# stone-d-chen/ffvvc

Measured on AMD Instinct MI355X. Metric: decoded frames/sec (4K/8K 10-bit VVC) per GPU, higher is better.
Workload: dtype u16

## Files before the change

ffvvc_amd/csrc/inter_cu.hip:

```cpp
#include <utility>

#include "common.hpp"
#include "inter_weight.hpp"
#include "runtime.hpp"
#include "../../include/vvc_mi355.h"
#include "stage_checks.hpp"

namespace vvc355 {

static_assert(sizeof(vvc355_affine_cu) == 144 && offsetof(vvc355_affine_cu, diff_mv) == 16 && offsetof(vvc355_affine_cu, first_job) == 12,
              "vvc355_affine_cu layout");
static_assert(sizeof(vvc355_gpm_cu) == 64 && offsetof(vvc355_gpm_cu, gpm_mv) == 16 && offsetof(vvc355_gpm_cu, first_job) == 12,
              "vvc355_gpm_cu layout");
static_assert(sizeof(vvc355_inter_frame) == 136, "vvc355_inter_frame layout");
static_assert(sizeof(vvc355_affine_frame) == 168 && offsetof(vvc355_affine_frame, cus) == 136 && offsetof(vvc355_affine_frame, n_cus) == 160,
              "vvc355_affine_frame layout");
static_assert(sizeof(vvc355_gpm_frame) == 160 && offsetof(vvc355_gpm_frame, cus) == 136 && offsetof(vvc355_gpm_frame, n_cus) == 152,
              "vvc355_gpm_frame layout");
static_assert(sizeof(vvc355_affine_job) == 96 && sizeof(vvc355_bipred_job) == 104 && sizeof(vvc355_gpm_job) == 120, "job layouts");
static_assert(sizeof(vvc355_ciip_cu) == 32 && offsetof(vvc355_ciip_cu, first_job) == 12 && offsetof(vvc355_ciip_cu, cmd) == 20, "vvc355_ciip_cu layout");
static_assert(sizeof(vvc355_ciip_frame) == 224 && offsetof(vvc355_ciip_frame, cus) == 136 && offsetof(vvc355_ciip_frame, n_cus) == 192 &&
              offsetof(vvc355_ciip_frame, ctb_log2) == 220, "vvc355_ciip_frame layout");
static_assert(sizeof(vvc355_recon_cmd) == 40 && offsetof(vvc355_recon_cmd, joint) == 33, "vvc355_recon_cmd layout");

void ciip_pred_launch(hipStream_t stream, int bd, const vvc355_bipred_job *jobs_dev, int n_jobs);

#define VVC355_TABLE(type, name, count) static constexpr type c_##name[count]
#include "tables_small.inc"
#undef VVC355_TABLE
#define VVC355_TABLE(type, name, count) __device__ static const type t_##name[count]
#include "tables_small.inc"
#undef VVC355_TABLE


constexpr int kGpmMaskSize = 112;
struct GpmMask { uint8_t w[kGpmMaskSize * kGpmMaskSize]; };

constexpr uint32_t gpm_used_angles()
{
    uint32_t m = 0;
    for (int p = 0; p < 64; p++) m |= 1u << c_gpm_angle_idx[p];
    return m;
}
constexpr uint32_t kGpmAngles = gpm_used_angles();
constexpr int kGpmMasks = __builtin_popcount(kGpmAngles);
static_assert(kGpmMasks == 20, "GPM uses 20 of the 32 angles");
__host__ __device__ constexpr int gpm_mask_slot(int angle) { return __builtin_popcount(kGpmAngles & ((1u << angle) - 1)); }
constexpr int gpm_slot_angle(int slot)
{
    for (int a = 0; a < 32; a++)
        if (((kGpmAngles >> a) & 1) && gpm_mask_slot(a) == slot) return a;
    return -1;
}

constexpr GpmMask make_gpm_mask(int angle)
{
    GpmMask m = {};
    const int dx = c_gpm_distance_lut[angle], dy = c_gpm_distance_lut[(angle + 8) % 32];
    const bool flip = !(angle >= 13 && angle <= 27);
    for (int v = 0; v < kGpmMaskSize; v++) {
        const int ry = (2 * (v - 56) + 1) * dy;
        for (int u = 0; u < kGpmMaskSize; u++) {
            const int idx = (2 * (u - 56) + 1) * dx + ry;
            const int s = ((flip ? 32 + idx : 32 - idx) + 4) >> 3;
            m.w[v * kGpmMaskSize + u] = (uint8_t)(s < 0 ? 0 : s > 8 ? 8 : s);
        }
    }
    return m;
}
template <int A> constexpr GpmMask kGpmMaskOf = make_gpm_mask(A);

template <typename Seq> struct GpmMaskSet;
template <size_t... S> struct GpmMaskSet<std::index_sequence<S...>> { GpmMask m[sizeof...(S)]; };
using GpmMaskTable = GpmMaskSet<std::make_index_sequence<kGpmMasks>>;
template <size_t... S> constexpr GpmMaskSet<std::index_sequence<S...>> make_gpm_masks(std::index_sequence<S...>)
{
    return { { kGpmMaskOf<gpm_slot_angle(S)>... } };
}
__device__ const GpmMaskTable d_gpm_masks = make_gpm_masks(std::make_index_sequence<kGpmMasks>{});
static const GpmMaskTable h_gpm_masks = make_gpm_masks(std::make_index_sequence<kGpmMasks>{});

struct GpmAddr { int slot, first, step_x, step_y; };
__host__ __device__ inline GpmAddr gpm_address(int angle, int distance, int cb_width, int cb_height, int hs, int vs)
{
    GpmAddr a;
    a.slot = gpm_mask_slot(angle);
    const bool shift_hor = !(angle % 16 == 8 || (angle % 16 != 0 && cb_height >= cb_width));
    int off_x = (-cb_width) >> 1, off_y = (-cb_height) >> 1;
    if (shift_hor)
        off_x += angle < 16 ? (distance * cb_width) >> 3 : -((distance * cb_width) >> 3);
    else
        off_y += angle < 16 ? (distance * cb_height) >> 3 : -((distance * cb_height) >> 3);
    const bool ok = cb_width >= 8 && cb_width <= 64 && cb_height >= 8 && cb_height <= 64 && ((kGpmAngles >> angle) & 1);
    a.first = ok ? (off_y + 56) * kGpmMaskSize + off_x + 56 : 0;
    a.step_x = ok ? 1 << hs : 0;
    a.step_y = ok ? kGpmMaskSize << vs : 0;
    return a;
}


template <typename Cu> __device__ __forceinline__ int find_cu(const Cu *cus, int n_cus, uint32_t i)
{
    int lo = 0, hi = n_cus - 1;
    while (lo < hi) {
        const int mid = (lo + hi + 1) >> 1;
        if (cus[mid].first_job <= i) lo = mid; else hi = mid - 1;
    }
    return lo;
}

__device__ __forceinline__ uint64_t plane_at(const vvc355_inter_frame &f, int c, int x, int y)
{
    return f.dst[c] + (uint64_t)y * f.dst_stride[c] + ((uint64_t)x << f.pixel_shift);
}

__device__ __forceinline__ int32_t round_mv_half(int32_t v) { return (v + 1 - (v >= 0)) >> 1; }

__global__ __launch_bounds__(256) void affine_build_kernel(const vvc355_affine_frame *__restrict__ fp)
{
    const vvc355_affine_frame F = load_uniform(fp);
    const vvc355_inter_frame &f = F.pic;
    const uint32_t i = blockIdx.x * blockDim.x + threadIdx.x;
    if (i >= (uint32_t)F.n_jobs)
        return;
    const vvc355_affine_cu *cus = (const vvc355_affine_cu *)F.cus;
    const int u = find_cu(cus, F.n_cus, i);
    const vvc355_affine_cu *cu = cus + u;
    const int x0 = cu->x0, y0 = cu->y0, cbw = cu->cb_width, cbh = cu->cb_height, nsx = cu->num_sb_x, nsy = cu->num_sb_y;
    const uint32_t first = cu->first_job;
    const uint32_t n_local = (u + 1 < F.n_cus ? cus[u + 1].first_job : (uint32_t)F.n_jobs) - first;
    const uint32_t k = i - first;
    const int hs = f.hs, vs = f.vs, csh = hs + vs;
    vvc355_affine_job *jl = (vvc355_affine_job *)F.jobs_luma;
    vvc355_bipred_job *jc = (vvc355_bipred_job *)F.jobs_chroma;
    const uint32_t cfirst = first >> csh;

    if (nsx != cbw >> 2 || nsy != cbh >> 2 || cbw < 8 || cbh < 8 || n_local != (uint32_t)(nsx * nsy)) {
        jl[i] = vvc355_affine_job{};
        if (f.chroma_format_idc && k < (n_local >> csh)) {
            jc[2 * (cfirst + k)] = vvc355_bipred_job{};
            jc[2 * (cfirst + k) + 1] = vvc355_bipred_job{};
        }
        return;
    }
    const vvc355_inter_slice *sl = (const vvc355_inter_slice *)f.slices + cu->slice;
    const vvc355_ref_pic *refs = (const vvc355_ref_pic *)f.refs;
    const MvFieldDev *mvf_tab = (const MvFieldDev *)f.mvf;
    const int sbx = k % nsx, sby = k / nsx;
    const int x = x0 + 4 * sbx, y = y0 + 4 * sby;
    const MvFieldDev mv = mvf_tab[(y >> 2) * f.mvf_stride + (x >> 2)];

    vvc355_affine_job j = {};
    j.dst = plane_at(f, 0, x, y);
    j.dst_stride = f.dst_stride[0];
    for (int l = 0; l < 2; l++) {
        if (!(mv.pred_flag & (1 << l)))
            continue;
        const vvc355_ref_pic rp = refs[l * 16 + mv.ref_idx[l]];
        (l ? j.ref1 : j.ref0) = rp.plane[0];
        (l ? j.ref1_stride : j.ref0_stride) = rp.stride[0];
        j.mv[2 * l] = mv.mv[l][0];
        j.mv[2 * l + 1] = mv.mv[l][1];
    }
    j.diff_mv = F.cus + (uint64_t)u * sizeof(vvc355_affine_cu) + offsetof(vvc355_affine_cu, diff_mv);
    j.x = (int16_t)x; j.y = (int16_t)y; j.pic_w = (int16_t)f.width; j.pic_h = (int16_t)f.height;
    set_pred_weight(j, derive_pred_weight(sl, mv, 0, false, false));
    j.pred_flag = mv.pred_flag;
    j.prof0 = cu->prof_flags & 1;
    j.prof1 = (cu->prof_flags >> 1) & 1;
    j.lmcs_lut = sl->lmcs_used ? f.lmcs_fwd_lut : 0;
    jl[i] = j;

    if (!f.chroma_format_idc || (sbx & ((1 << hs) - 1)) || (sby & ((1 << vs) - 1)))
        return;
    const MvFieldDev mv2 = mvf_tab[((y + vs * 4) >> 2) * f.mvf_stride + ((x + hs * 4) >> 2)];
    MvFieldDev mvc = mv;
    for (int l = 0; l < 2; l++)
        for (int d = 0; d < 2; d++)
// ... 82 lines not shown
    const vvc355_inter_frame &f = F.pic;
    const uint32_t i = blockIdx.x * blockDim.x + threadIdx.x;
    if (i >= (uint32_t)F.n_jobs)
        return;
    vvc355_bipred_job *slot = (vvc355_bipred_job *)F.jobs + i;
    vvc355_bipred_job j = {};
    const vvc355_ciip_cu *cus = (const vvc355_ciip_cu *)F.cus;
    const int u = find_cu(cus, F.n_cus, i);
    const vvc355_ciip_cu cu = cus[u];
    const int x0 = cu.x0, y0 = cu.y0, cbw = cu.cb_width, cbh = cu.cb_height, ctb_log2 = F.ctb_log2;
    const bool side_ok = cbw >= 4 && cbw <= 64 && !(cbw & (cbw - 1)) && cbh >= 4 && cbh <= 64 && !(cbh & (cbh - 1)) && cbw * cbh >= 64;
    const bool inside = x0 >= 0 && y0 >= 0 && !((x0 | y0) & 3) && x0 + cbw <= f.width && y0 + cbh <= f.height &&
                        (x0 >> ctb_log2) == ((x0 + cbw - 1) >> ctb_log2) && (y0 >> ctb_log2) == ((y0 + cbh - 1) >> ctb_log2);
    const bool has_c = f.chroma_format_idc != 0;
    const int wc = cbw >> f.hs, hc = cbh >> f.vs;
    const bool blend_c = has_c && wc > 2;
    const uint32_t ntl = ((cbw + 15) >> 4) * ((cbh + 15) >> 4), ntc = has_c ? ((wc + 15) >> 4) * ((hc + 15) >> 4) : 0;
    const uint32_t region = cbw * cbh + (blend_c ? 2 * wc * hc : 0);
    uint32_t k = i - cu.first_job;
    if (!side_ok || !inside || i < cu.first_job || cu.slice >= F.n_slices || (uint64_t)cu.first_job + ntl + 2 * ntc > (uint64_t)(uint32_t)F.n_jobs ||
        (uint64_t)cu.scratch_off + region > (uint64_t)(uint32_t)F.scratch_len || k >= ntl + 2 * ntc) {
        *slot = j;
        return;
    }
    const MvFieldDev *mvf_tab = (const MvFieldDev *)f.mvf;
    const MvFieldDev mv = mvf_tab[(y0 >> 2) * f.mvf_stride + (x0 >> 2)];
    bool mv_ok = mv.pred_flag >= 1 && mv.pred_flag <= 3;
    for (int l = 0; l < 2; l++)
        mv_ok = mv_ok && (!(mv.pred_flag & (1 << l)) || (mv.ref_idx[l] >= 0 && mv.ref_idx[l] <= 15));
    if (!mv_ok) {
        *slot = j;
        return;
    }
    const vvc355_inter_slice *sl = (const vvc355_inter_slice *)f.slices + cu.slice;
    const vvc355_ref_pic *refs = (const vvc355_ref_pic *)f.refs;
    int c = 0;
    if (k >= ntl) {
        k -= ntl;
        c = 1;
        if (k >= ntc) { k -= ntc; c = 2; }
    }
    const int hs = c ? f.hs : 0, vs = c ? f.vs : 0;
    const int w = cbw >> hs, h = cbh >> vs, tw = min(w, 16), th = min(h, 16);
    const int ntx = (w + 15) >> 4;
    const int tx = (k % ntx) * tw, ty = (k / ntx) * th;
    const int x = (x0 >> hs) + tx, y = (y0 >> vs) + ty;
    const bool to_plane = c && !blend_c;
    const uint64_t part = F.scratch + (((uint64_t)cu.scratch_off + (c ? cbw * cbh + (c - 1) * wc * hc : 0)) << f.pixel_shift);

    if (to_plane) {
        j.dst_stride = c == 1 ? f.dst_stride[1] : f.dst_stride[2];
        j.dst = (c == 1 ? f.dst[1] : f.dst[2]) + (uint64_t)y * j.dst_stride + ((uint64_t)x << f.pixel_shift);
    } else {
        j.dst = part + ((uint64_t)(ty * w + tx) << f.pixel_shift);
        j.dst_stride = w << f.pixel_shift;
    }
    for (int l = 0; l < 2; l++) {
        if (!(mv.pred_flag & (1 << l)))
            continue;
        const vvc355_ref_pic *rp = refs + l * 16 + mv.ref_idx[l];
        (l ? j.ref1 : j.ref0) = rp->plane[c];
        (l ? j.ref1_stride : j.ref0_stride) = rp->stride[c];
        j.mv[2 * l] = mv.mv[l][0];
        j.mv[2 * l + 1] = mv.mv[l][1];
    }
    j.x = (int16_t)x; j.y = (int16_t)y; j.w = (int16_t)tw; j.h = (int16_t)th;
    j.pic_w = (int16_t)(f.width >> hs); j.pic_h = (int16_t)(f.height >> vs);
    j.chroma = c > 0; j.hs = f.hs; j.vs = f.vs;
    j.hf_idx = j.vf_idx = c ? 0 : cu.hpel_if_idx & 1;
    j.pred_flag = mv.pred_flag;
    j.lmcs_lut = (!c && sl->lmcs_used) ? f.lmcs_fwd_lut : 0;
    set_pred_weight(j, derive_pred_weight(sl, mv, c, false, true));
    *slot = j;

    if (!F.cmds || k || to_plane)
        return;
    const uint32_t ci = cus[u].cmd[c];
    if (ci >= (uint32_t)F.n_cmds)
        return;
    vvc355_recon_cmd *cmd = (vvc355_recon_cmd *)F.cmds + ci;
    if (cmd->kind != VVC355_RECON_CIIP || cmd->c_idx != c || cmd->x0 != x0 || cmd->y0 != y0 || cmd->w != cbw || cmd->h != cbh)
        return;
    const int16_t *slice_idx = (const int16_t *)F.slice_idx, *col_bd = (const int16_t *)F.ctb_to_col_bd, *row_bd = (const int16_t *)F.ctb_to_row_bd;
    const int rx = x0 >> ctb_log2, ry = y0 >> ctb_log2, ncx = F.ctb_width, rs = ry * ncx + rx, ctb_mask = (1 << ctb_log2) - 1;
    const bool left_tile = rx > 0 && col_bd[rx] != col_bd[rx - 1];
    const bool upper_tile = ry > 0 && row_bd[ry] != row_bd[ry - 1];
    const bool upper_slice = ry > 0 && slice_idx[rs] != slice_idx[rs - ncx];
    const bool ctb_left = rx > 0 && !left_tile, ctb_up = ry > 0 && !upper_tile && !upper_slice;
    const bool available_l = ctb_left || (x0 & ctb_mask), available_u = ctb_up || (y0 & ctb_mask);
    int weight = 1;
    if (available_u && mvf_tab[((y0 - 1) >> 2) * f.mvf_stride + ((x0 - 1 + cbw) >> 2)].pred_flag == 0)
        weight++;
    if (available_l && mvf_tab[((y0 - 1 + cbh) >> 2) * f.mvf_stride + ((x0 - 1) >> 2)].pred_flag == 0)
        weight++;
    cmd->resid = part;
    cmd->joint = (uint8_t)weight;
}

int ciip_frame_check(const vvc355_ciip_frame *F, int bd)
{
    if (!F)
        return VVC355_CIIP_E_FRAME;
    const vvc355_inter_frame &f = F->pic;
    if (f.width <= 0 || f.height <= 0 || (f.width & 3) || (f.height & 3))
        return VVC355_CIIP_E_SIZE;
    if (F->ctb_log2 < 5 || F->ctb_log2 > 7)
        return VVC355_CIIP_E_CTB;
    const int ctb = 1 << F->ctb_log2;
    if (F->ctb_width != (f.width + ctb - 1) >> F->ctb_log2 || F->ctb_height != (f.height + ctb - 1) >> F->ctb_log2)
        return VVC355_CIIP_E_GRID;
    if (F->n_cus < 0 || F->n_jobs < 0 || F->scratch_len < 0 || F->n_slices < 0 || F->n_cmds < 0)
        return VVC355_CIIP_E_COUNT;
    if (bd >= 0 && ((bd != 8 && bd != 10 && bd != 12) || f.pixel_shift != (bd > 8)))
        return VVC355_CIIP_E_DEPTH;
    if (bd < 0 && f.pixel_shift > 1)
        return VVC355_CIIP_E_DEPTH;
    const int fmt_hs[4] = { 0, 1, 1, 0 }, fmt_vs[4] = { 0, 1, 0, 0 };
    if (f.chroma_format_idc > 3 || f.hs != fmt_hs[f.chroma_format_idc] || f.vs != fmt_vs[f.chroma_format_idc])
        return VVC355_CIIP_E_FORMAT;
    if (F->n_cus > 0 && !F->cus)
        return VVC355_CIIP_E_RECORDS;
    if (F->n_jobs > 0 && !F->jobs)
        return VVC355_CIIP_E_JOBS;
    if (!F->scratch || !f.mvf || !f.refs || !f.slices || !f.dst[0] || (f.chroma_format_idc && (!f.dst[1] || !f.dst[2])) || f.mvf_stride < f.width / 4)
        return VVC355_CIIP_E_TABLES;
    if (F->cmds && (!F->slice_idx || !F->ctb_to_col_bd || !F->ctb_to_row_bd))
        return VVC355_CIIP_E_CMDS;
    return 0;
}

}

extern "C" {

void vvc355_affine_frame_build(void *stream, const vvc355_affine_frame *frame_dev, const vvc355_affine_frame *frame_host)
{
    if (frame_host->n_cus <= 0 || frame_host->n_jobs <= 0) return;
    hipLaunchKernelGGL(vvc355::affine_build_kernel, dim3((frame_host->n_jobs + 255) / 256), dim3(256), 0, (hipStream_t)stream, frame_dev);
    HIP_CHECK(hipGetLastError());
}

void vvc355_affine_frame_pass(void *stream, int bd, const vvc355_affine_frame *frame_dev, const vvc355_affine_frame *frame_host)
{
    if (frame_host->n_cus <= 0 || frame_host->n_jobs <= 0) return;
    vvc355_affine_frame_build(stream, frame_dev, frame_host);
    vvc355_affine_frame_predict(stream, bd, frame_dev, frame_host);
}

void vvc355_affine_frame_predict(void *stream, int bd, const vvc355_affine_frame *, const vvc355_affine_frame *frame_host)
{
    if (frame_host->n_cus <= 0 || frame_host->n_jobs <= 0) return;
    vvc355_affine_batch(stream, bd, (const vvc355_affine_job *)frame_host->jobs_luma, frame_host->n_jobs);
    if (frame_host->pic.chroma_format_idc)
        vvc355_bipred_chroma_batch(stream, bd, (const vvc355_bipred_job *)frame_host->jobs_chroma,
                                   2 * (frame_host->n_jobs >> (frame_host->pic.hs + frame_host->pic.vs)));
}

void vvc355_gpm_frame_build(void *stream, const vvc355_gpm_frame *frame_dev, const vvc355_gpm_frame *frame_host)
{
    if (frame_host->n_cus <= 0 || frame_host->n_jobs <= 0) return;
    hipLaunchKernelGGL(vvc355::gpm_build_kernel, dim3((frame_host->n_jobs + 255) / 256), dim3(256), 0, (hipStream_t)stream, frame_dev);
    HIP_CHECK(hipGetLastError());
}

void vvc355_gpm_frame_pass(void *stream, int bd, const vvc355_gpm_frame *frame_dev, const vvc355_gpm_frame *frame_host)
{
    if (frame_host->n_cus <= 0 || frame_host->n_jobs <= 0) return;
    vvc355_gpm_frame_build(stream, frame_dev, frame_host);
    vvc355_gpm_frame_predict(stream, bd, frame_dev, frame_host);
}

void vvc355_gpm_frame_predict(void *stream, int bd, const vvc355_gpm_frame *, const vvc355_gpm_frame *frame_host)
{
    if (frame_host->n_cus <= 0 || frame_host->n_jobs <= 0) return;
    vvc355_gpm_batch(stream, bd, (const vvc355_gpm_job *)frame_host->jobs, frame_host->n_jobs);
}

int vvc355_ciip_frame_build(void *stream, const vvc355_ciip_frame *frame_dev, const vvc355_ciip_frame *frame_host)
{
    const int err = frame_dev ? vvc355::ciip_frame_check(frame_host, -1) : VVC355_CIIP_E_FRAME;
    if (err)
        return err;
    if (frame_host->n_cus == 0 || frame_host->n_jobs == 0) return 0;
    hipLaunchKernelGGL(vvc355::ciip_build_kernel, dim3((frame_host->n_jobs + 255) / 256), dim3(256), 0, (hipStream_t)stream, frame_dev);
    HIP_CHECK(hipGetLastError());
    return 0;
}

int vvc355_ciip_frame_pass(void *stream, int bd, const vvc355_ciip_frame *frame_dev, const vvc355_ciip_frame *frame_host)
{
    const int err = frame_dev ? vvc355::ciip_frame_check(frame_host, bd) : VVC355_CIIP_E_FRAME;
    if (err)
        return err;
    if (frame_host->n_cus == 0 || frame_host->n_jobs == 0) return 0;
    vvc355_ciip_frame_build(stream, frame_dev, frame_host);
    return vvc355_ciip_frame_predict(stream, bd, frame_dev, frame_host);
}

int vvc355_ciip_frame_predict(void *stream, int bd, const vvc355_ciip_frame *frame_dev, const vvc355_ciip_frame *frame_host)
{
    const int err = frame_dev ? vvc355::ciip_frame_check(frame_host, bd) : VVC355_CIIP_E_FRAME;
    if (err)
        return err;
    if (frame_host->n_cus == 0 || frame_host->n_jobs == 0) return 0;
    vvc355::ciip_pred_launch((hipStream_t)stream, bd, (const vvc355_bipred_job *)frame_host->jobs, frame_host->n_jobs);
    return 0;
}

void vvc355_gpm_weights(int partition_idx, int cb_width, int cb_height, int hs, int vs, uint8_t *out)
{
    using namespace vvc355;
    const int part = partition_idx & 63;
    const GpmAddr a = gpm_address(c_gpm_angle_idx[part], c_gpm_distance_idx[part], cb_width, cb_height, hs, vs);
    const uint8_t *m = h_gpm_masks.m[a.slot].w;
    const int w = cb_width >> hs, h = cb_height >> vs;
    for (int y = 0; y < h; y++)
        for (int x = 0; x < w; x++)
            out[y * w + x] = m[a.first + y * a.step_y + x * a.step_x];
}

}
```

ffvvc_amd/csrc/mc_fused.hip:

```cpp
#include <type_traits>
#include "common.hpp"
#include "runtime.hpp"
#include "../../include/vvc_mi355.h"

namespace vvc355 {

#define VVC355_TABLE(type, name, count) __device__ static const type d_tab_##name[count]
#include "tables.inc"
#undef VVC355_TABLE

typedef short v2s __attribute__((ext_vector_type(2)));

__device__ __forceinline__ int dot2(uint32_t a, uint32_t b, int acc)
{
    return __builtin_amdgcn_sdot2(__builtin_bit_cast(v2s, a), __builtin_bit_cast(v2s, b), acc, false);
}
__device__ __forceinline__ uint32_t pack16(int lo, int hi) { return (uint32_t)(lo & 0xffff) | ((uint32_t)hi << 16); }
__device__ __forceinline__ int tap_of(uint32_t lo, uint32_t hi, int k)
{
    const uint32_t v = k < 4 ? lo : hi;
    return (int)(int8_t)(v >> ((k & 3) * 8));
}

static constexpr int kWinW = 24;
// ... 320 lines not shown
            uint16_t r0[NIT], r1[NIT];
            fetch_clamped<BD, NIT>(pa, sa, g.rc[0], ax, ay, lane, r0);
            if (both)
                fetch_clamped<BD, NIT>(pb, sb, g.rc[1], bx, by, lane, r1);
            store_rows<NIT>(L.win[0], lane, r0);
            if (both)
                store_rows<NIT>(L.win[1], lane, r1);
        }
        wave_sync();
    }
    uint32_t t[2][4];
#pragma unroll
    for (int i = 0; i < 2; i++) {
        if (NTAP == 8) {
            const uint2 hf = gld<uint2>(d_tab_inter_luma_filters + (job->hf_idx * 16 + g.fx[i]) * 8);
            const uint2 vf = gld<uint2>(d_tab_inter_luma_filters + (job->vf_idx * 16 + g.fy[i]) * 8);
            t[i][0] = hf.x; t[i][1] = hf.y; t[i][2] = vf.x; t[i][3] = vf.y;
        } else {
            t[i][0] = gld<uint32_t>(d_tab_inter_chroma_filters + (job->hf_idx * 32 + g.fx[i]) * 4); t[i][1] = 0;
            t[i][2] = gld<uint32_t>(d_tab_inter_chroma_filters + (job->vf_idx * 32 + g.fy[i]) * 4); t[i][3] = 0;
        }
    }
    interp_block<BD, NTAP>(lw, h, g.fx[0] != 0, g.fy[0] != 0, t[0][0], t[0][1], t[0][2], t[0][3], L.win[0], L.tmpT, lane, v0);
    if (both)
        interp_block<BD, NTAP>(lw, h, g.fx[1] != 0, g.fy[1] != 0, t[1][0], t[1][1], t[1][2], t[1][3], L.win[1], L.tmpT, lane, v1);
    else {
#pragma unroll
        for (int i = 0; i < 4; i++) v1[i] = 0;
    }
}

#include "mc_tools.hpp"

union BipredLdsAll {
    BipredLds plain;
    ToolsLds<16, 16> tools;
};

template <int BD>
__device__ __forceinline__ void bipred_plain(const vvc355_bipred_job *job, BipredLds &L, int lane, const vvc355_gpm_job *gpm = nullptr)
{
    const int uni = job->pred_flag == 1 || job->pred_flag == 2;
    const int w = job->w, h = job->h, chroma = job->chroma;
    const int lw = 31 - __builtin_clz(w);
    vvc355_bipred_result *rec = (vvc355_bipred_result *)job->rec;
    int mv[4] = { job->mv[0], job->mv[1], job->mv[2], job->mv[3] };
    if (rec && chroma) {
#pragma unroll
        for (int k = 0; k < 4; k++) mv[k] = gld<int>(&rec->mv[k]);
    } else if (rec && lane == 0) {
#pragma unroll
        for (int k = 0; k < 4; k++) gst<int>(&rec->mv[k], mv[k]);
        gst<int>(&rec->bdof, 0);
        gst<int>(&rec->min_sad, 0);
        gst<int>(&rec->searched, 0);
    }
    RefGeom g = ref_geometry(job, mv, chroma, chroma && job->dmvr && !uni);
    const uint8_t *lut = chroma ? nullptr : (const uint8_t *)job->lmcs_lut;
    int v0[4], v1[4];
    const uint8_t *pa = (const uint8_t *)job->ref0, *pb = (const uint8_t *)job->ref1;
    int sa = job->ref0_stride, sb = job->ref1_stride;
    if (uni && job->pred_flag == 2) {
        pa = pb; sa = sb;
        g.ox[0] = g.ox[1]; g.oy[0] = g.oy[1]; g.fx[0] = g.fx[1]; g.fy[0] = g.fy[1]; g.rc[0] = g.rc[1];
    }
    if (chroma)
        predict_clamped<BD, 4>(job, L, lane, lw, h, g, v0, v1, pa, sa, pb, sb, !uni);
    else
        predict_clamped<BD, 8>(job, L, lane, lw, h, g, v0, v1, pa, sa, pb, sb, !uni);
    if (uni) {
        const int wfu = job->weight_flag, sh = (wfu ? job->denom : 0) + 14 - BD, rnd = 1 << (sh - 1);
        const int xu = lane & 15;
        uint8_t *dstu = (uint8_t *)job->dst;
#pragma unroll
        for (int i = 0; i < 4; i++) {
            const int y = 2 * ((lane >> 4) + 4 * (i >> 1)) + (i & 1);
            if (xu >= w || y >= h)
                continue;
            const int p = wfu ? ((v0[i] * job->w0 + rnd) >> sh) + job->o0 * (1 << (BD - 8)) : (v0[i] + rnd) >> sh;
            gst_at<typename Px<BD>::type>(dstu, (uint32_t)(__mul24(y, job->dst_stride) + xu * (int)sizeof(typename Px<BD>::type)), (typename Px<BD>::type)lmcs_fwd<BD>(lut, clip_px<BD>(p)));
        }
        return;
    }
#pragma unroll
    for (int i = 0; i < 4; i++) { v0[i] = (int16_t)v0[i]; v1[i] = (int16_t)v1[i]; }
    if (gpm) {
        constexpr int gsh = BD <= 12 ? 17 - BD : 5, goff = 1 << (gsh - 1);
        const uint8_t *wt = (const uint8_t *)gpm->weights;
        const int xg = lane & 15;
        uint8_t *dstg = (uint8_t *)job->dst;
#pragma unroll
        for (int i = 0; i < 4; i++) {
            const int y = 2 * ((lane >> 4) + 4 * (i >> 1)) + (i & 1);
            if (xg >= w || y >= h)
                continue;
            const int wg = gld<uint8_t>(wt + y * gpm->step_y + xg * gpm->step_x);
            const int p = (v0[i] * wg + v1[i] * (8 - wg) + goff) >> gsh;
            gst_at<typename Px<BD>::type>(dstg, (uint32_t)(__mul24(y, job->dst_stride) + xg * (int)sizeof(typename Px<BD>::type)), (typename Px<BD>::type)lmcs_fwd<BD>(lut, clip_px<BD>(p)));
        }
        return;
    }
    int shift, off;
    const int wf = job->weight_flag, w0 = job->w0, w1 = job->w1;
    if (!wf) { shift = max(3, 15 - BD); off = 1 << (shift - 1); }
    else     { shift = job->denom + max(3, 15 - BD); off = (((job->o0 + job->o1) << (BD - 8)) + 1) << (shift - 1); }
    const int x = lane & 15;
    uint8_t *dst = (uint8_t *)job->dst;
#pragma unroll
    for (int i = 0; i < 4; i++) {
        const int y = 2 * ((lane >> 4) + 4 * (i >> 1)) + (i & 1);
        if (x >= w || y >= h)
            continue;
        const int p = wf ? (v0[i] * w0 + v1[i] * w1 + off) >> shift : (v0[i] + v1[i] + off) >> shift;
        gst_at<typename Px<BD>::type>(dst, (uint32_t)(__mul24(y, job->dst_stride) + x * (int)sizeof(typename Px<BD>::type)), (typename Px<BD>::type)lmcs_fwd<BD>(lut, clip_px<BD>(p)));
    }
}

template <int BD, bool TOOLS>
__global__ __launch_bounds__(256) void bipred_kernel(const vvc355_bipred_job *__restrict__ jobs, int n_jobs)
{
    __shared__ __attribute__((aligned(16))) BipredLdsAll lds_all[4];
    const int wave = __builtin_amdgcn_readfirstlane(threadIdx.x >> 6), lane = threadIdx.x & 63;
    const int ji = xcd_chunked(blockIdx.x, gridDim.x) * 4 + wave;
    if (ji >= n_jobs)
        return;
    const vvc355_bipred_job job_copy = load_uniform(jobs + ji);
    const vvc355_bipred_job *job = &job_copy;
    BipredLdsAll &L = lds_all[wave];
    const int w = job->w, h = job->h, uni = job->pred_flag == 1 || job->pred_flag == 2;
    if (TOOLS && !job->chroma && !uni && (job->dmvr || job->bdof) && (w == 8 || w == 16) && (h == 8 || h == 16)) {
        if (w == 16 && h == 16)     bipred_tools<BD, 16, 16>(job, L.tools, lane);
        else if (w == 16)           bipred_tools<BD, 16, 8>(job, *(ToolsLds<16, 8> *)&L.tools, lane);
        else if (h == 16)           bipred_tools<BD, 8, 16>(job, *(ToolsLds<8, 16> *)&L.tools, lane);
        else                        bipred_tools<BD, 8, 8>(job, *(ToolsLds<8, 8> *)&L.tools, lane);
        return;
    }
    bipred_plain<BD>(job, L.plain, lane);
}

template <int BD>
__global__ __launch_bounds__(256) void gpm_kernel(const vvc355_gpm_job *__restrict__ jobs, int n_jobs)
{
    __shared__ __attribute__((aligned(16))) BipredLds lds_all[4];
    const int wave = __builtin_amdgcn_readfirstlane(threadIdx.x >> 6), lane = threadIdx.x & 63;
    const int ji = xcd_chunked(blockIdx.x, gridDim.x) * 4 + wave;
    if (ji >= n_jobs)
        return;
    const vvc355_gpm_job job = load_uniform(jobs + ji);
    vvc355_bipred_job base = job.base;
    base.pred_flag = 3; base.dmvr = 0; base.bdof = 0; base.weight_flag = 0; base.rec = 0;
    bipred_plain<BD>(&base, lds_all[wave], lane, &job);
}

template <int BD>
__global__ __launch_bounds__(256) void bipred_chroma_pair_kernel(const vvc355_bipred_job *__restrict__ jobs, int n_jobs)
{
    __shared__ __attribute__((aligned(16))) BipredLds lds_all[4];
    using px_t = typename Px<BD>::type;
    const int wave = __builtin_amdgcn_readfirstlane(threadIdx.x >> 6), lane = threadIdx.x & 63;
    const int ia = 2 * (xcd_chunked(blockIdx.x, gridDim.x) * 4 + wave);
    if (ia >= n_jobs)
        return;
    const bool has_b = ia + 1 < n_jobs;
    const vvc355_bipred_job ja = load_uniform(jobs + ia), jb = load_uniform(jobs + (has_b ? ia + 1 : ia));
    BipredLds &L = lds_all[wave];
    const bool bi_a = !(ja.pred_flag == 1 || ja.pred_flag == 2), bi_b = !(jb.pred_flag == 1 || jb.pred_flag == 2);
    bool pair = has_b && bi_a && bi_b && ja.chroma && jb.chroma && ja.w <= 8 && ja.w == jb.w && ja.h == jb.h && ja.x == jb.x && ja.y == jb.y &&
                ja.rec == jb.rec && ja.hs == jb.hs && ja.vs == jb.vs && ja.dmvr == jb.dmvr && ja.hf_idx == jb.hf_idx &&
                ja.vf_idx == jb.vf_idx && ja.pic_w == jb.pic_w && ja.pic_h == jb.pic_h;
#pragma unroll
    for (int k = 0; k < 4; k++) pair = pair && ja.mv[k] == jb.mv[k];
    if (!pair) {
        if (ja.chroma)
            bipred_plain<BD>(&ja, L, lane);
        if (has_b && jb.chroma) {
            wave_sync();
            bipred_plain<BD>(&jb, L, lane);
        }
        return;
    }
    const vvc355_bipred_job *job = &ja;
    const int w = job->w, h = job->h;
    const vvc355_bipred_result *rec = (const vvc355_bipred_result *)job->rec;
    int mv[4] = { job->mv[0], job->mv[1], job->mv[2], job->mv[3] };
    if (rec) {
#pragma unroll
        for (int k = 0; k < 4; k++) mv[k] = rec->mv[k];
    }
    const RefGeom g = ref_geometry(job, mv, true, job->dmvr);
    {
        const int c = lane & 31, second = c >= 12, cc = c - (second ? 12 : 0);
        uint16_t r[2][10];
#pragma unroll
        for (int i = 0; i < 2; i++) {
            const uint8_t *pa = (const uint8_t *)(i ? ja.ref1 : ja.ref0), *pb = (const uint8_t *)(i ? jb.ref1 : jb.ref0);
            const int sa = i ? ja.ref1_stride : ja.ref0_stride, sb = i ? jb.ref1_stride : jb.ref0_stride;
            const uint8_t *plane = second ? pb : pa;
            const int stride = second ? sb : sa;
            const int xa = clip3(g.ox[i] - 1 + cc, g.rc[i].x0, g.rc[i].x1);
            const uint8_t *col = plane + xa * (int)sizeof(px_t);
            const int wy0 = g.oy[i] - (g.fy[i] ? 1 : 0);
#pragma unroll
            for (int it = 0; it < 10; it++) {
                const int ya = clip3(wy0 + (lane >> 5) + 2 * it, g.rc[i].y0, g.rc[i].y1);
                r[i][it] = (uint16_t)gld<px_t>(col + row_off(ya, stride));
            }
        }
        store_rows<10>(L.win[0], lane, r[0]);
        store_rows<10>(L.win[1], lane, r[1]);
        wave_sync();
    }
    uint32_t t[2][2];
#pragma unroll
    for (int i = 0; i < 2; i++) {
        t[i][0] = gld<uint32_t>(d_tab_inter_chroma_filters + (job->hf_idx * 32 + g.fx[i]) * 4);
        t[i][1] = gld<uint32_t>(d_tab_inter_chroma_filters + (job->vf_idx * 32 + g.fy[i]) * 4);
    }
    int v0[4], v1[4];
    interp_block<BD, 4, true>(4, h, g.fx[0] != 0, g.fy[0] != 0, t[0][0], 0, t[0][1], 0, L.win[0], L.tmpT, lane, v0);
    interp_block<BD, 4, true>(4, h, g.fx[1] != 0, g.fy[1] != 0, t[1][0], 0, t[1][1], 0, L.win[1], L.tmpT, lane, v1);
#pragma unroll
    for (int i = 0; i < 4; i++) { v0[i] = (int16_t)v0[i]; v1[i] = (int16_t)v1[i]; }
    const int x = lane & 15, second = x >= 8, xo = x - (second ? 8 : 0);
    const int wf = second ? jb.weight_flag : ja.weight_flag, w0 = second ? jb.w0 : ja.w0, w1 = second ? jb.w1 : ja.w1;
    const int denom = second ? jb.denom : ja.denom, osum = second ? jb.o0 + jb.o1 : ja.o0 + ja.o1;
    const int shift = wf ? denom + max(3, 15 - BD) : max(3, 15 - BD);
    const int off = wf ? ((osum << (BD - 8)) + 1) << (shift - 1) : 1 << (shift - 1);
    uint8_t *dst = (uint8_t *)(second ? jb.dst : ja.dst);
    const int dst_stride = second ? jb.dst_stride : ja.dst_stride;
#pragma unroll
    for (int i = 0; i < 4; i++) {
        const int y = 2 * ((lane >> 4) + 4 * (i >> 1)) + (i & 1);
        if (xo >= w || y >= h)
            continue;
        const int p = wf ? (v0[i] * w0 + v1[i] * w1 + off) >> shift : (v0[i] + v1[i] + off) >> shift;
        st_px<BD>(dst + row_off(y, dst_stride), xo, clip_px<BD>(p));
    }
}

template <int BD>
__global__ __launch_bounds__(256) void ciip_pred_kernel(const vvc355_bipred_job *__restrict__ jobs, int n_jobs)
{
    __shared__ __attribute__((aligned(16))) BipredLds lds_all[4];
    const int wave = __builtin_amdgcn_readfirstlane(threadIdx.x >> 6), lane = threadIdx.x & 63;
    const int ji = xcd_chunked(blockIdx.x, gridDim.x) * 4 + wave;
    if (ji >= n_jobs)
        return;
    const vvc355_bipred_job job = load_uniform(jobs + ji);
    if (job.w <= 0 || job.h <= 0)
        return;
    bipred_plain<BD>(&job, lds_all[wave], lane);
}

}

extern "C" void vvc355_pred_fused_batch(void *stream, int bd, const vvc355_pred_job *jobs_dev, int n_jobs)
{
    using namespace vvc355;
    if (n_jobs <= 0) return;
    VVC355_BD_DISPATCH(bd, hipLaunchKernelGGL((pred_fused_kernel<BD>), dim3((n_jobs + 3) / 4), dim3(256), 0, (hipStream_t)stream, jobs_dev, n_jobs));
    HIP_CHECK(hipGetLastError());
}

extern "C" void vvc355_bipred_batch(void *stream, int bd, const vvc355_bipred_job *jobs_dev, int n_jobs)
{
    using namespace vvc355;
    if (n_jobs <= 0) return;
    VVC355_BD_DISPATCH(bd, hipLaunchKernelGGL((bipred_kernel<BD, true>), dim3((n_jobs + 3) / 4), dim3(256), 0, (hipStream_t)stream, jobs_dev, n_jobs));
    HIP_CHECK(hipGetLastError());
}

extern "C" void vvc355_gpm_batch(void *stream, int bd, const vvc355_gpm_job *jobs_dev, int n_jobs)
{
    using namespace vvc355;
    if (n_jobs <= 0) return;
    VVC355_BD_DISPATCH(bd, hipLaunchKernelGGL((gpm_kernel<BD>), dim3((n_jobs + 3) / 4), dim3(256), 0, (hipStream_t)stream, jobs_dev, n_jobs));
    HIP_CHECK(hipGetLastError());
}

extern "C" void vvc355_bipred_chroma_batch(void *stream, int bd, const vvc355_bipred_job *jobs_dev, int n_jobs)
{
    using namespace vvc355;
    if (n_jobs <= 0) return;
    const int n_pairs = (n_jobs + 1) / 2;
    VVC355_BD_DISPATCH(bd, hipLaunchKernelGGL((bipred_chroma_pair_kernel<BD>), dim3((n_pairs + 3) / 4), dim3(256), 0, (hipStream_t)stream, jobs_dev, n_jobs));
    HIP_CHECK(hipGetLastError());
}

namespace vvc355 {

void ciip_pred_launch(hipStream_t stream, int bd, const vvc355_bipred_job *jobs_dev, int n_jobs)
{
    if (n_jobs <= 0) return;
    VVC355_BD_DISPATCH(bd, hipLaunchKernelGGL((ciip_pred_kernel<BD>), dim3((n_jobs + 3) / 4), dim3(256), 0, stream, jobs_dev, n_jobs));
    HIP_CHECK(hipGetLastError());
}

}
```

Measured before the change: 552.2.

## Add quad chroma path processing four 8x8 Cb/Cr pairs per wave

After: 561.7 (median of 6 runs). +1.7%, better.

```diff
diff --git a/ffvvc_amd/csrc/inter_cu.hip b/ffvvc_amd/csrc/inter_cu.hip
--- a/ffvvc_amd/csrc/inter_cu.hip
+++ b/ffvvc_amd/csrc/inter_cu.hip
@@ -24,6 +24,7 @@
 static_assert(sizeof(vvc355_recon_cmd) == 40 && offsetof(vvc355_recon_cmd, joint) == 33, "vvc355_recon_cmd layout");
 
 void ciip_pred_launch(hipStream_t stream, int bd, const vvc355_bipred_job *jobs_dev, int n_jobs);
+void chroma_pairs_launch(hipStream_t stream, int bd, const vvc355_bipred_job *jobs_dev, int n_jobs);
 
 #define VVC355_TABLE(type, name, count) static constexpr type c_##name[count]
 #include "tables_small.inc"
@@ -412,8 +413,8 @@
     if (frame_host->n_cus <= 0 || frame_host->n_jobs <= 0) return;
     vvc355_affine_batch(stream, bd, (const vvc355_affine_job *)frame_host->jobs_luma, frame_host->n_jobs);
     if (frame_host->pic.chroma_format_idc)
-        vvc355_bipred_chroma_batch(stream, bd, (const vvc355_bipred_job *)frame_host->jobs_chroma,
-                                   2 * (frame_host->n_jobs >> (frame_host->pic.hs + frame_host->pic.vs)));
+        vvc355::chroma_pairs_launch((hipStream_t)stream, bd, (const vvc355_bipred_job *)frame_host->jobs_chroma,
+                                    2 * (frame_host->n_jobs >> (frame_host->pic.hs + frame_host->pic.vs)));
 }
 
 void vvc355_gpm_frame_build(void *stream, const vvc355_gpm_frame *frame_dev, const vvc355_gpm_frame *frame_host)
diff --git a/ffvvc_amd/csrc/mc_chroma_quad.hpp b/ffvvc_amd/csrc/mc_chroma_quad.hpp
--- /dev/null
+++ b/ffvvc_amd/csrc/mc_chroma_quad.hpp
@@ -0,0 +1,183 @@
+#pragma once
+
+static constexpr int kQwP = 20;
+static constexpr int kQwC0 = 4;
+static constexpr int kQwRows = 11;
+static constexpr int kQtP = 16;
+
+struct QuadGroupLds {
+    union {
+        uint16_t win[4][kQwRows * kQwP];
+        int16_t tmpT[4][8 * kQtP];
+    };
+};
+struct QuadLds { QuadGroupLds g[4]; };
+
+struct QuadTaps {
+    uint32_t a[3], b[3];
+    __device__ __forceinline__ void set(uint32_t f4, bool odd)
+    {
+        const int f0 = (int8_t)f4, f1 = (int8_t)(f4 >> 8), f2 = (int8_t)(f4 >> 16), f3 = (int8_t)(f4 >> 24);
+        const uint32_t e0 = pack16(f0, f1), e1 = pack16(f2, f3);
+        const uint32_t o0 = pack16(0, f0), o1 = pack16(f1, f2), o2 = pack16(f3, 0);
+        a[0] = odd ? o0 : e0; a[1] = odd ? o1 : e1; a[2] = odd ? o2 : 0u;
+        b[0] = odd ? 0u : o0; b[1] = odd ? e0 : o1; b[2] = odd ? e1 : o2;
+    }
+    __device__ __forceinline__ void apply(uint32_t d0, uint32_t d1, uint32_t d2, int &out0, int &out1) const
+    {
+        out0 = dot2(d2, a[2], dot2(d1, a[1], dot2(d0, a[0], 0)));
+        out1 = dot2(d2, b[2], dot2(d1, b[1], dot2(d0, b[0], 0)));
+    }
+};
+
+__device__ __forceinline__ int lo16s(uint32_t v) { return (int)(int16_t)(v & 0xffff); }
+__device__ __forceinline__ int hi16s(uint32_t v) { return (int)v >> 16; }
+__device__ __forceinline__ const uint8_t *ptr64(uint32_t lo, uint32_t hi) { return (const uint8_t *)(((uint64_t)hi << 32) | lo); }
+
+template <int BD>
+__device__ __forceinline__ bool chroma_quad(const vvc355_bipred_job *jobs, int ia, QuadLds &LQ, int lane)
+{
+    using px_t = typename Px<BD>::type;
+    static_assert(sizeof(vvc355_bipred_job) == 104, "descriptor layout: dword indices below");
+#define VVC355_QUAD_AT(field, byte) static_assert(offsetof(vvc355_bipred_job, field) == (byte), "descriptor layout: " #field)
+    VVC355_QUAD_AT(dst, 0); VVC355_QUAD_AT(ref0, 8); VVC355_QUAD_AT(ref1, 16); VVC355_QUAD_AT(rec, 24);
+    VVC355_QUAD_AT(dst_stride, 32); VVC355_QUAD_AT(ref0_stride, 36); VVC355_QUAD_AT(ref1_stride, 40); VVC355_QUAD_AT(mv, 44);
+    VVC355_QUAD_AT(x, 60); VVC355_QUAD_AT(y, 62); VVC355_QUAD_AT(w, 64); VVC355_QUAD_AT(h, 66); VVC355_QUAD_AT(pic_w, 68); VVC355_QUAD_AT(pic_h, 70);
+    VVC355_QUAD_AT(denom, 72); VVC355_QUAD_AT(w0, 74); VVC355_QUAD_AT(w1, 76); VVC355_QUAD_AT(o0, 78); VVC355_QUAD_AT(o1, 80);
+    VVC355_QUAD_AT(chroma, 82); VVC355_QUAD_AT(hs, 83); VVC355_QUAD_AT(vs, 84); VVC355_QUAD_AT(dmvr, 85); VVC355_QUAD_AT(bdof, 86);
+    VVC355_QUAD_AT(hf_idx, 87); VVC355_QUAD_AT(vf_idx, 88); VVC355_QUAD_AT(weight_flag, 89); VVC355_QUAD_AT(pred_flag, 90);
+#undef VVC355_QUAD_AT
+    const int grp = lane >> 4, l = lane & 15;
+
+    uint32_t a[24], b[24];
+    {
+        const uint8_t *pa = (const uint8_t *)(jobs + ia + 2 * grp), *pb = pa + sizeof(vvc355_bipred_job);
+#pragma unroll
+        for (int i = 0; i < 12; i++) {
+            const uint2 va = gld<uint2>(pa + 8 * i), vb = gld<uint2>(pb + 8 * i);
+            a[2 * i] = va.x; a[2 * i + 1] = va.y;
+            b[2 * i] = vb.x; b[2 * i + 1] = vb.y;
+        }
+    }
+    bool ok = a[6] == b[6] && a[7] == b[7];
+#pragma unroll
+    for (int k = 11; k <= 17; k++) ok = ok && a[k] == b[k];
+    const uint32_t pfa = (a[22] >> 16) & 0xff, pfb = (b[22] >> 16) & 0xff;
+    ok = ok && ((a[20] ^ b[20]) >> 16) == 0 && ((a[20] >> 16) & 0xff) != 0 && (a[20] >> 24) == 1 &&
+         ((a[21] ^ b[21]) & 0xff00ffffu) == 0 && (a[21] & 0xff) == 1 &&
+         ((a[22] ^ b[22]) & 0xff) == 0 &&
+         !(pfa == 1 || pfa == 2) && !(pfb == 1 || pfb == 2) && a[16] == (8u | (8u << 16));
+
+    int mv[4] = { (int)a[11], (int)a[12], (int)a[13], (int)a[14] };
+    const uint8_t *rec = ptr64(a[6], a[7]);
+    if (ok && rec) {
+#pragma unroll
+        for (int k = 0; k < 4; k++) mv[k] = gld<int>(rec + 4 * k);
+    }
+    const int x = lo16s(a[15]), y = hi16s(a[15]), pic_w = lo16s(a[17]), pic_h = hi16s(a[17]);
+    const bool dmvr = ((a[21] >> 8) & 0xff) != 0;
+    int bx[2], by[2], dx[2], dy[2];
+#pragma unroll
+    for (int i = 0; i < 2; i++) {
+        const int ox = x + (mv[2 * i] >> 5), oy = y + (mv[2 * i + 1] >> 5);
+        bx[i] = dmvr ? x + ((int)a[11 + 2 * i] >> 5) : ox;
+        by[i] = dmvr ? y + ((int)a[12 + 2 * i] >> 5) : oy;
+        dx[i] = ox - bx[i];
+        dy[i] = oy - by[i];
+        ok = ok && (unsigned)(dx[i] + 2) <= 4u && (unsigned)(dy[i] + 2) <= 4u &&
+             bx[i] >= 1 && bx[i] + 10 < pic_w && by[i] >= 1 && by[i] + 9 < pic_h;
+    }
+    if (!__all(ok))
+        return false;
+
+    QuadGroupLds &L = LQ.g[grp];
+    const int q = l >> 2, ref = q >> 1, second = q & 1;
+    {
+        const int k = l & 3;
+        const uint8_t *plane = second ? (ref ? ptr64(b[4], b[5]) : ptr64(b[2], b[3])) : (ref ? ptr64(a[4], a[5]) : ptr64(a[2], a[3]));
+        const int stride = (int)(second ? (ref ? b[10] : b[9]) : (ref ? a[10] : a[9]));
+        const int fx0 = (ref ? bx[1] : bx[0]) - 1 + 4 * min(k, 2), fy0 = (ref ? by[1] : by[0]) - 1;
+        const uint8_t *p = plane + row_off(fy0, stride) + fx0 * (int)sizeof(px_t);
+        uint2 v[kQwRows];
+#pragma unroll
+        for (int r = 0; r < kQwRows; r++) {
+            if (BD > 8) {
+                v[r] = gld<uint2>(p);
+            } else {
+                const uint32_t s = gld<uint32_t>(p);
+                v[r] = make_uint2(__builtin_amdgcn_perm(0, s, 0x0c010c00u), __builtin_amdgcn_perm(0, s, 0x0c030c02u));
+            }
+            p += stride;
+        }
+        uint16_t *wq = L.win[q] + kQwC0 + 4 * k;
+#pragma unroll
+        for (int r = 0; r < kQwRows; r++) {
+            uint2 d = v[r];
+            const uint32_t rep = __builtin_amdgcn_perm(0, d.y, 0x01000100u);
+            if (k >= 2) d.y = rep;
+            if (k == 3) d.x = rep;
+            *(uint2 *)(wq + r * kQwP) = d;
+            if (k == 0)
+                *(uint32_t *)(wq + r * kQwP - 2) = __builtin_amdgcn_perm(0, d.x, 0x01000100u);
+        }
+        wave_sync();
+    }
+    const uint32_t hf_idx = a[21] >> 24, vf_idx = a[22] & 0xff;
+
+    {
+        const int xp = l & 3, d = ref ? dx[1] : dx[0], fx = (ref ? mv[2] : mv[0]) & 31;
+        QuadTaps t;
+        t.set(gld<uint32_t>(d_tab_inter_chroma_filters + (fx ? hf_idx * 32 + fx : 0) * 4), d & 1);
+        const uint32_t *rp = (const uint32_t *)(L.win[q] + 2 * xp + kQwC0 + d - (d & 1));
+        int t0[kQwRows], t1[kQwRows];
+#pragma unroll
+        for (int r = 0; r < kQwRows; r++) {
+            int o0, o1;
+            t.apply(rp[r * (kQwP / 2)], rp[r * (kQwP / 2) + 1], rp[r * (kQwP / 2) + 2], o0, o1);
+            t0[r] = o0 >> (BD - 8);
+            t1[r] = o1 >> (BD - 8);
+        }
+        wave_sync();
+        uint4 *c0 = (uint4 *)(L.tmpT[q] + (2 * xp) * kQtP), *c1 = (uint4 *)(L.tmpT[q] + (2 * xp + 1) * kQtP);
+        c0[0] = make_uint4(pack16(t0[0], t0[0]), pack16(t0[0], t0[1]), pack16(t0[2], t0[3]), pack16(t0[4], t0[5]));
+        c0[1] = make_uint4(pack16(t0[6], t0[7]), pack16(t0[8], t0[9]), pack16(t0[10], t0[10]), pack16(t0[10], t0[10]));
+        c1[0] = make_uint4(pack16(t1[0], t1[0]), pack16(t1[0], t1[1]), pack16(t1[2], t1[3]), pack16(t1[4], t1[5]));
+        c1[1] = make_uint4(pack16(t1[6], t1[7]), pack16(t1[8], t1[9]), pack16(t1[10], t1[10]), pack16(t1[10], t1[10]));
+        wave_sync();
+    }
+
+    const int pl = l >> 3, xo = l & 7;
+    int val[2][8];
+#pragma unroll
+    for (int i = 0; i < 2; i++) {
+        const int d = dy[i], fy = mv[2 * i + 1] & 31;
+        QuadTaps t;
+        t.set(gld<uint32_t>(d_tab_inter_chroma_filters + (fy ? vf_idx * 32 + fy : 0) * 4), d & 1);
+        const uint32_t *cp = (const uint32_t *)(L.tmpT[2 * i + pl] + xo * kQtP + 2 + d - (d & 1));
+        uint32_t c[6];
+#pragma unroll
+        for (int m = 0; m < 6; m++) c[m] = cp[m];
+#pragma unroll
+        for (int yp = 0; yp < 4; yp++) {
+            int o0, o1;
+            t.apply(c[yp], c[yp + 1], c[yp + 2], o0, o1);
+            val[i][2 * yp] = (int16_t)(o0 >> 6);
+            val[i][2 * yp + 1] = (int16_t)(o1 >> 6);
+        }
+    }
+
+    const uint32_t s18 = pl ? b[18] : a[18], s19 = pl ? b[19] : a[19], s20 = pl ? b[20] : a[20], s22 = pl ? b[22] : a[22];
+    const bool wf = ((s22 >> 8) & 0xff) != 0;
+    const int denom = wf ? lo16s(s18) : 0, w0 = wf ? hi16s(s18) : 1, w1 = wf ? lo16s(s19) : 1;
+    const int osum = wf ? hi16s(s19) + lo16s(s20) : 0;
+    const int shift = denom + max(3, 15 - BD);
+    const int off = ((osum << (BD - 8)) + 1) << (shift - 1);
+    uint8_t *dst = (uint8_t *)(pl ? ptr64(b[0], b[1]) : ptr64(a[0], a[1]));
+    const int dst_stride = (int)(pl ? b[8] : a[8]);
+#pragma unroll
+    for (int yy = 0; yy < 8; yy++) {
+        const int p = (val[0][yy] * w0 + val[1][yy] * w1 + off) >> shift;
+        st_px<BD>(dst + row_off(yy, dst_stride), xo, clip_px<BD>(p));
+    }
+    return true;
+}
diff --git a/ffvvc_amd/csrc/mc_fused.hip b/ffvvc_amd/csrc/mc_fused.hip
--- a/ffvvc_amd/csrc/mc_fused.hip
+++ b/ffvvc_amd/csrc/mc_fused.hip
@@ -496,18 +496,14 @@
     bipred_plain<BD>(&base, lds_all[wave], lane, &job);
 }
 
+#include "mc_chroma_quad.hpp"
+
 template <int BD>
-__global__ __launch_bounds__(256) void bipred_chroma_pair_kernel(const vvc355_bipred_job *__restrict__ jobs, int n_jobs)
-{
-    __shared__ __attribute__((aligned(16))) BipredLds lds_all[4];
+__device__ __forceinline__ void chroma_pair(const vvc355_bipred_job *__restrict__ jobs, int ia, int n_jobs, BipredLds &L, int lane)
+{
     using px_t = typename Px<BD>::type;
-    const int wave = __builtin_amdgcn_readfirstlane(threadIdx.x >> 6), lane = threadIdx.x & 63;
-    const int ia = 2 * (xcd_chunked(blockIdx.x, gridDim.x) * 4 + wave);
-    if (ia >= n_jobs)
-        return;
     const bool has_b = ia + 1 < n_jobs;
     const vvc355_bipred_job ja = load_uniform(jobs + ia), jb = load_uniform(jobs + (has_b ? ia + 1 : ia));
-    BipredLds &L = lds_all[wave];
     const bool bi_a = !(ja.pred_flag == 1 || ja.pred_flag == 2), bi_b = !(jb.pred_flag == 1 || jb.pred_flag == 2);
     bool pair = has_b && bi_a && bi_b && ja.chroma && jb.chroma && ja.w <= 8 && ja.w == jb.w && ja.h == jb.h && ja.x == jb.x && ja.y == jb.y &&
                 ja.rec == jb.rec && ja.hs == jb.hs && ja.vs == jb.vs && ja.dmvr == jb.dmvr && ja.hf_idx == jb.hf_idx &&
@@ -582,6 +578,45 @@
     }
 }
 
+union ChromaLds {
+    BipredLds plain;
+    QuadLds quad;
+};
+
+template <int BD>
+__global__ __launch_bounds__(128) __attribute__((amdgpu_waves_per_eu(5, 5))) void bipred_chroma_pair_kernel(const vvc355_bipred_job *__restrict__ jobs, int n_jobs)
+{
+    __shared__ __attribute__((aligned(16))) ChromaLds lds_all[2];
+    const int wave = __builtin_amdgcn_readfirstlane(threadIdx.x >> 6), lane = threadIdx.x & 63;
+    const int ia = 8 * (xcd_chunked(blockIdx.x, gridDim.x) * 2 + wave);
+    if (ia >= n_jobs)
+        return;
+    ChromaLds &L = lds_all[wave];
+    if (ia + 8 <= n_jobs) {
+        const vvc355_bipred_job j0 = load_uniform(jobs + ia);
+        if (j0.w == 8 && j0.h == 8 && j0.hs == 1 && j0.vs == 1 && j0.chroma && j0.pred_flag != 1 && j0.pred_flag != 2 &&
+            chroma_quad<BD>(jobs, ia, L.quad, lane))
+            return;
+    }
+    const int end = min(ia + 8, n_jobs);
+#pragma unroll 1
+    for (int i = ia; i < end; i += 2) {
+        chroma_pair<BD>(jobs, i, n_jobs, L.plain, lane);
+        wave_sync();
+    }
+}
+
+template <int BD>
+__global__ __launch_bounds__(256) void bipred_chroma_one_pair_kernel(const vvc355_bipred_job *__restrict__ jobs, int n_jobs)
+{
+    __shared__ __attribute__((aligned(16))) BipredLds lds_all[4];
+    const int wave = __builtin_amdgcn_readfirstlane(threadIdx.x >> 6), lane = threadIdx.x & 63;
+    const int ia = 2 * (xcd_chunked(blockIdx.x, gridDim.x) * 4 + wave);
+    if (ia >= n_jobs)
+        return;
+    chroma_pair<BD>(jobs, ia, n_jobs, lds_all[wave], lane);
+}
+
 template <int BD>
 __global__ __launch_bounds__(256) void ciip_pred_kernel(const vvc355_bipred_job *__restrict__ jobs, int n_jobs)
 {
@@ -626,12 +661,20 @@
 {
     using namespace vvc355;
     if (n_jobs <= 0) return;
+    const int n_waves = (n_jobs + 7) / 8;
+    VVC355_BD_DISPATCH(bd, hipLaunchKernelGGL((bipred_chroma_pair_kernel<BD>), dim3((n_waves + 1) / 2), dim3(128), 0, (hipStream_t)stream, jobs_dev, n_jobs));
+    HIP_CHECK(hipGetLastError());
+}
+
+namespace vvc355 {
+
+void chroma_pairs_launch(hipStream_t stream, int bd, const vvc355_bipred_job *jobs_dev, int n_jobs)
+{
+    if (n_jobs <= 0) return;
     const int n_pairs = (n_jobs + 1) / 2;
-    VVC355_BD_DISPATCH(bd, hipLaunchKernelGGL((bipred_chroma_pair_kernel<BD>), dim3((n_pairs + 3) / 4), dim3(256), 0, (hipStream_t)stream, jobs_dev, n_jobs));
+    VVC355_BD_DISPATCH(bd, hipLaunchKernelGGL((bipred_chroma_one_pair_kernel<BD>), dim3((n_pairs + 3) / 4), dim3(256), 0, stream, jobs_dev, n_jobs));
     HIP_CHECK(hipGetLastError());
 }
-
-namespace vvc355 {
 
 void ciip_pred_launch(hipStream_t stream, int bd, const vvc355_bipred_job *jobs_dev, int n_jobs)
 {
```
